# NVIDIA/tensorrt-laboratory

Hardware: NVIDIA H100
Metric: ResNet-50 fp16 b=8 inferences/sec (higher is better)
Workload: dtype f16

## Files before the change

__graft_entry__.py:

```python
from __future__ import annotations

import os
import re
import shutil
import subprocess
import sysconfig
import sys

ROOT = os.path.dirname(os.path.abspath(__file__))
PKG = os.path.join(ROOT, "tensorrt_laboratory_b200")
CSRC = os.path.join(PKG, "csrc")
LIB = os.path.join(PKG, "libb200infer.so")

NVCC_FLAGS = [
    "-gencode", "arch=compute_90a,code=sm_90a", "-lineinfo", "-O3", "-std=c++17",
    "-Xcompiler", "-fPIC,-Wall,-Wno-unused-function", "-cudart", "static",
]


def _nvcc() -> str:
    for cand in (os.environ.get("NVCC"), shutil.which("nvcc"), "/usr/local/cuda/bin/nvcc"):
        if cand and os.path.exists(cand):
            return cand
    raise RuntimeError("nvcc not found")
# ... 20 lines not shown

def _all_deps():
    deps = []
    for root, _, files in os.walk(CSRC):
        deps += [os.path.join(root, f) for f in files if f.endswith((".cu", ".cc", ".h", ".cuh", ".hpp"))]
    deps.append(os.path.join(ROOT, "include", "b200infer.h"))
    inc = os.path.join(ROOT, "include")
    for root, _, files in os.walk(inc):
        deps += [os.path.join(root, f) for f in files]
    return deps


_CONV_KERNEL = re.compile(r"conv|net_f16_tcgen05|attention_f16_wgmma|embed_ln|layernorm_h8|pooler")


_SHARED_SM_KERNEL = re.compile(r"_ZN3b2k(?:16conv_f16_tcgen05|20conv3x3_halo_tcgen05)ILi(\d+)E")
_SHARED_SM_THREADS = 320


def _shared_sm_register_budget(bn: int):
    ctas = 3 if bn <= 64 else 2 if bn <= 128 else 1
    return None if ctas == 1 else 65536 // (_SHARED_SM_THREADS * ctas) // 8 * 8


def _ptxas_violations(log: str):
    bad = [line.strip() for line in log.splitlines() if "(C7520)" in line or "(C7518)" in line]
    func = None
    for line in log.splitlines():
        m = re.search(r"Function properties for (\S+)", line)
        if m:
            func = m.group(1)
# ... 93 lines not shown
```

tensorrt_laboratory_b200/csrc/engine.cu:

```cuda
#include <cuda.h>
#include <cuda_runtime.h>
#include <stdarg.h>
#include <stdio.h>
#include <stdlib.h>
#include <string.h>

#include <algorithm>
#include <map>
#include <memory>
#include <mutex>
#include <string>
#include <vector>

#include "../../include/b200infer.h"
#include "kernels.h"
#include "plan_format.h"

#include "b2_internal.h"

namespace b2i {
thread_local std::string g_err;
int fail(int code, const char* fmt, ...) {
    char buf[1024];
    va_list ap;
// ... 237 lines not shown
    uint8_t* scratch = nullptr;
    struct ScratchState {
        std::map<int, std::unique_ptr<Plan>> plans;
    };
    std::map<uint8_t*, ScratchState> states;
    ScratchState* cur = nullptr;
    int* d_counters = nullptr;
    int use_graph = 1;
    int force_simt = 0;
    int force_im2col = 0;
    int force_bn = 0;
    int force_stages = 0;
    int force_splits = 0;
    int force_sps = 0;
    int force_halo = 0;
    int force_cn = 0;
    int force_ws = 0;
    int pdl_trigger = 1;
    int no_fold = 0;
    int autotune = 4;
    int fork = 0;
    int net = 0;
    int net_ctas = 0;
    int net_bn = 0;
    int net_stages = 0;
    int i8_bn = 0;
    int i8_stages = 0;
    int fuse_tail = 1;
    int input_ctas = 0;
    int* d_tail_ctrl = nullptr;
// ... 301 lines not shown
            return fail(B2_EINVAL, "plan: tactic table outside the blob");
        for (uint32_t i = 0; i < h.n_tactics; ++i) {
            TacticRec t;
            memcpy(&t, base + h.tactics_offset + size_t(i) * sizeof(TacticRec), sizeof t);
            if (t.op >= h.n_ops || t.batch == 0 || t.batch > h.max_batch) return fail(B2_EINVAL, "plan: tactic %u out of range", i);
            ConvConfig cfg{int(t.bn), int(t.stages), int(t.splits), 0.0, int(t.sps), int(t.ws), int(t.cn)};
            cfg.halo = int(t.halo);
            e->tuned[{int(t.op), int(t.batch)}] = cfg;
        }
        e->tactics_from_plan = true;
    }
    *payload = base + h.payload_offset;
    return B2_OK;
}

void plan_arena(b2_engine* e) {
    int busy_until = -1;
    for (size_t i = 0; i < e->ops.size(); ++i) {
        Op& op = e->ops[i];
        op.side_join = -1;
        if (int(i) <= busy_until || op.r.type != b2plan::OP_CONV || op.r.out < 0 || e->tensors[op.r.out].binding >= 0) continue;
        int consumers = 0, join = -1;
        bool as_residual_only = true;
        for (size_t k = i + 1; k < e->ops.size(); ++k) {
            const auto& rk = e->ops[k].r;
            if (rk.in == op.r.out) ++consumers, as_residual_only = false;
            if (rk.res == op.r.out) ++consumers, join = int(k);
        }
        if (consumers == 1 && as_residual_only && join > int(i) + 1) {
            op.side_join = join;
            busy_until = join;
        }
    }
    for (size_t i = 0; i < e->ops.size(); ++i) {
        const auto& r = e->ops[i].r;
        for (int t : {r.out, e->ops[i].out2})
            if (t >= 0 && e->tensors[t].def < 0) e->tensors[t].def = int(i);
        for (int t : {r.in, r.res})
            if (t >= 0) e->tensors[t].last_use = std::max(e->tensors[t].last_use, int(i));
        if (e->ops[i].side_join >= 0 && r.in >= 0) e->tensors[r.in].last_use = std::max(e->tensors[r.in].last_use, e->ops[i].side_join);
    }
    struct Live {
        size_t off, size;
        int last;
    };
    std::vector<Live> live;
    size_t top = 0;
    std::vector<int> order;
    for (size_t i = 0; i < e->tensors.size(); ++i)
        if (e->tensors[i].binding < 0 && e->tensors[i].def >= 0) order.push_back(int(i));
    std::stable_sort(order.begin(), order.end(), [&](int a, int b) { return e->tensors[a].def < e->tensors[b].def; });
    for (int ti : order) {
        Tensor& t = e->tensors[ti];
        if (t.last_use < t.def) t.last_use = t.def;
        const size_t size = align_up(t.item_bytes * e->max_batch, 1024);
// ... 108 lines not shown
    const b2plan::OpRec& r = op.r;
    return !c->no_fold && r.cin_phys == 8 && op.kw() * 8 * 2 == 64 && op.sw() == 1 && op.pw_lo() == 0 && op.pw_hi() == 0;
}
int conv_kb(const b2_context* c, const Op& op) {
    if (op.r.cin_phys % 64 == 0) return 64;
    return conv_is_row_folded(c, op) ? 32 : 8;
}
int conv_num_kblocks(const b2_context* c, const Op& op) {
    const b2plan::OpRec& r = op.r;
    if (op.group_span()) return int(r.taps) * (op.group_span() / 64);
    if (r.cin_phys % 64 == 0) return int(r.taps) * (int(r.cin_phys) / 64);
    if (conv_is_row_folded(c, op)) return (op.kh() + 1) / 2;
    return (int(r.taps_phys) + 7) / 8;
}

int conv_halo_rows(const b2_context* c, const Op& op) {
    const b2plan::OpRec& r = op.r;
    const Tensor& ti = c->e->tensors[r.in];
    const Tensor& to = c->e->tensors[r.out];
    if (op.groups > 1 || r.cin_phys % 64 || r.cout_phys % 64 || op.kh() != 3 || op.kw() != 3 || op.sh() != 1 || op.sw() != 1 || op.ph() != 1 ||
        op.pw_lo() != 1 || op.pw_hi() != 1 || r.res >= 0 || !(r.relu & 2) || ti.h != to.h || ti.w != to.w)
        return 0;
    const int wp = int(to.w) + 2;
    if (wp > 128) return 0;
    return std::min(128 / wp, int(to.h));
}

bool conv_on_tensor_cores(const b2_engine* e, const Op& op) {
    const b2plan::OpRec& r = op.r;
    const bool kb64 = r.cin_phys % 64 == 0, kb8 = r.cin_phys == 8;
    return e->half() && (kb64 || kb8) && r.cout_phys % 32 == 0 && (kb64 || r.taps_phys % 2 == 0) && (op.groups == 1 || op.group_span() > 0);
}

bool conv_takes_stem_ws(const b2_context* c, const Op& op) {
    const b2plan::OpRec& r = op.r;
    return conv_is_row_folded(c, op) && op.kh() == 7 && op.sh() == 2 && r.cout_phys == 64 && c->e->tensors[r.out].w <= 128 &&
           (r.relu & b2plan::kConvRelu) && !(r.relu & 2) && !(r.relu & b2plan::kConvGelu) && r.res < 0 && op.groups == 1;
}

bool conv_takes_ws(const b2_context* c, const Op& op) {
    return conv_takes_stem_ws(c, op) || (conv_kb(c, op) == 64 && (op.r.relu & 2) && op.groups == 1 && !(op.r.relu & b2plan::kConvGelu));
}

bool tactic_applies(const b2_context* c, const Op& op, int batch, const ConvConfig& cfg) {
    const b2plan::OpRec& r = op.r;
    const Tensor& to = c->e->tensors[r.out];
    const int span = op.group_span(), kb = conv_kb(c, op);
    if (cfg.bn <= 0 || int(r.cout_phys) % cfg.bn || cfg.splits < 1 || cfg.sps < 1 || cfg.ws < 0) return false;
    if (op.groups > 1 && (!span || span % cfg.bn || cfg.splits > 1)) return false;
    if ((op.groups > 1 || (r.relu & b2plan::kConvGelu)) && (cfg.ws || cfg.cn > 1 || cfg.halo)) return false;
    if (cfg.halo) {
        const int R = conv_halo_rows(c, op), cblocks = int(r.cin_phys) / 64;
        return R && cfg.splits == 1 && !cfg.ws && cfg.cn <= 1 && b2k::conv_halo_config_exists(cfg.bn) && cblocks <= 8 &&
               b2k::conv_halo_smem(cfg.bn, int(to.w), R, cblocks) <= kSmemLimit;
    }
    if (cfg.ws && conv_is_row_folded(c, op))
        return conv_takes_stem_ws(c, op) && cfg.bn == 64 && cfg.stages == b2k::kStemWsRing && cfg.sps == 1 && cfg.splits == 1 &&
               cfg.cn <= 1 && b2k::conv_stem_ws_smem() <= kSmemLimit;
    if (cfg.ws)
        return conv_takes_ws(c, op) && cfg.splits == 1 && cfg.cn <= 1 && b2k::conv_ws_config_exists(cfg.bn, cfg.stages, cfg.sps) &&
               b2k::conv_ws_smem(cfg.bn, cfg.stages, cfg.sps, r.res >= 0) <= kSmemLimit;
    if (!b2k::conv_config_exists(cfg.bn, kb, cfg.stages, cfg.sps) || b2k::conv_smem_bytes(cfg.bn, cfg.stages, r.res >= 0, cfg.sps) > kSmemLimit)
        return false;
    const int grid_n = int(r.cout_phys) / cfg.bn;
    if (cfg.cn > 1 && (kb != 64 || grid_n % cfg.cn || !b2k::conv_cluster_config_exists(cfg.bn, cfg.stages, cfg.sps, cfg.cn))) return false;
    if (cfg.splits > 1) {
        const int nkb = conv_num_kblocks(c, op), kpc = (nkb + cfg.splits - 1) / cfg.splits;
        const int tiles = (batch * int(to.h * to.w) + 127) / 128 * grid_n;
        if (kb != 64 || kpc < 4 || (cfg.splits - 1) * kpc >= nkb || tiles > kMaxSplitTiles ||
            size_t(tiles) * cfg.splits * 128 * cfg.bn * 4 > kSplitWorkspaceBytes)
            return false;
    }
    return true;
}

std::vector<ConvConfig> conv_candidates(const b2_context* c, const Op& op, int batch, int fixed_splits) {
    const b2plan::OpRec& r = op.r;
    const int kbsz = conv_kb(c, op), nkb = conv_num_kblocks(c, op);
    const int m_tiles = (batch * int(c->e->tensors[r.out].h * c->e->tensors[r.out].w) + 127) / 128;
    const bool ws_only = c->force_ws > 0 && conv_takes_ws(c, op);
    auto ok = [&](const ConvConfig& t) { return tactic_applies(c, op, batch, t); };
    std::vector<ConvConfig> out;
    for (int bn : {256, 128, 64, 32}) {
        if (int(r.cout_phys) % bn) continue;
        const int tiles = m_tiles * (int(r.cout_phys) / bn);
        for (int ws = 0; ws <= 1; ++ws)
        for (int sp : {1, 2, 4, 8})
        for (int sps = 1; sps <= 2; ++sps)
// ... 115 lines not shown
    a.pad_h = op.ph();
    a.pad_w = op.pw_lo();
    a.relu = int(r.relu & (b2plan::kConvRelu | b2plan::kConvGelu));
    a.wpacked = (r.relu & 2) ? w : nullptr;
    const bool tiled = r.k == 1 && op.kw() == 1 && r.stride == 1 && op.sw() == 1 && r.pad_ == 0 && op.pw_lo() == 0 &&
                       op.pw_hi() == 0 && kb64 && (!c->force_im2col || gelu);
    a.a_mode = tiled ? b2k::A_TILED : b2k::A_IM2COL;
    if (cfg.halo) {
        const int R = conv_halo_rows(c, op);
        cl.halo = 1;
        cl.ws_ctas = 0, cl.cn = 1, a.cn = 1, a.splits = 1, cl.stages = kHaloStagesTag, cl.sps = 1;
        a.halo_rows = R;
        cl.grid_m = batch * ((int(to.h) + R - 1) / R);
        int rc = make_map_nhwc(&cl.mapA, tptr(r.in), int(r.cin_phys), int(ti.w), int(ti.h), batch, uint32_t(ti.w) + 2, uint32_t(R) + 2);
        if (rc) return rc;
        rc = make_map_nhwc(&cl.mapOut, tptr(r.out), int(r.cout_phys), int(to.w), int(to.h), batch, uint32_t(to.w) + 2, uint32_t(R));
        cl.mapB = cl.mapA, cl.mapRes = cl.mapOut;
        return rc;
    }
    const CUtensorMapSwizzle swz = kb64 ? CU_TENSOR_MAP_SWIZZLE_128B : (fold ? CU_TENSOR_MAP_SWIZZLE_64B : CU_TENSOR_MAP_SWIZZLE_NONE);
    const uint64_t pix = uint64_t(r.cin_phys) * 2, rowb = uint64_t(ti.w) * pix, imgb = uint64_t(ti.h) * rowb;
    int rc;
    if (tiled)
        rc = make_map_2d(&cl.mapA, tptr(r.in), r.cin_phys, uint64_t(M), 64, uint32_t(128 / cl.cn), swz);
    else if (fold)
        rc = make_map_im2col(&cl.mapA, tptr(r.in), int(r.cin_phys) * op.kw(), int(ti.w) - op.kw() + 1, int(ti.h), batch, pix,
                             rowb, imgb, op.kh(), 1, op.sh(), 1, op.ph(), 0, 0, 32, 128, swz);
    else
        rc = make_map_im2col(&cl.mapA, tptr(r.in), int(r.cin_phys), int(ti.w), int(ti.h), batch, pix, rowb, imgb, op.kh(),
                             op.kw(), op.sh(), op.sw(), op.ph(), op.pw_lo(), op.pw_hi(), uint32_t(cl.kb), uint32_t(128 / cl.cn), swz);
    if (rc) return rc;
    if (r.relu & 2)
// ... 264 lines not shown
        const bool no_split = side || op.groups > 1;
        static const bool tune_splitk = env_int("B2_TUNE_SPLITK", 0) != 0;
        int splits = (no_split || !tune_splitk) ? 1 : 0;
        if (batch != e->max_batch && !no_split && tune_splitk) {
            std::lock_guard<std::mutex> lock(e->tune_mutex);
            auto it = e->tuned.find({int(i), e->max_batch});
            if (it != e->tuned.end()) splits = it->second.splits;
        }
        ConvConfig cfg = pick_conv_config(batch * int(to.h) * int(to.w), int(r.cout_phys), nkb, kbsz, r.res >= 0, c, false,
                                          op.group_span());
        int rc = autotune_conv(c, op, batch, splits, &cfg);
        if (rc) return rc;
        std::lock_guard<std::mutex> lock(e->tune_mutex);
        e->tuned[{int(i), batch}] = cfg;
        tune_cache_append(e, int(i), batch, cfg);
    }
    return B2_OK;
}

int fuse_net_runs(b2_context* c, Plan* plan, int batch) {
    b2_engine* e = c->e;
    std::vector<Launch>& ls = plan->launches;
    bool any = false;
    for (const Launch& L : ls) any = any || L.net_member;
    if (!any) return B2_OK;
    std::vector<Launch> fused;
    size_t i = 0;
    while (i < ls.size()) {
        if (!ls[i].net_member) {
            fused.push_back(std::move(ls[i]));
// ... 110 lines not shown
        run->ctas = std::max(1, std::min(run->ctas, std::min(2 * g_sms, tile_cursor)));
        run->first_op = int(i), run->last_op = int(j);
        Launch L;
        L.kind = L_NET;
        L.name = ls[i].name + ".." + ls[j].name;
        L.flops = flops, L.bytes = bytes;
        L.N = batch;
        L.net = run;
        fused.push_back(std::move(L));
        i = j + 1;
    }
    for (Launch& L : fused) L.side_join = -1;
    ls = std::move(fused);
    plan->has_net = true;
    return B2_OK;
}

void fuse_tail(b2_context* c, Plan* plan, int batch) {
    if (!c->fuse_tail || !c->e->half()) return;
    std::vector<Launch>& ls = plan->launches;
    for (size_t i = 0; i + 2 < ls.size(); ++i) {
        const Launch &P = ls[i], &F = ls[i + 1], &S = ls[i + 2];
        if (P.kind != L_AVGPOOL || F.kind != L_FC || S.kind != L_SOFTMAX) continue;
        if (F.in != P.out || S.in != F.out || F.out_binding >= 0 || S.in_binding >= 0 || S.out_binding < 0 || P.C_phys % 8) continue;
        if (F.K != P.C_phys || S.C != F.Cout || !b2k::tail_f16_applies(batch, P.H * P.W, P.C_phys, F.Cout)) continue;
        Launch T;
        T.kind = L_TAIL;
        T.name = P.name + "+" + F.name + "+" + S.name;
        T.N = batch;
        T.flops = F.flops, T.bytes = P.bytes + F.bytes + S.bytes;
// ... 112 lines not shown
                                        c->force_ws <= 0 && c->force_cn <= 0 && c->force_halo <= 0 && !c->force_im2col && op.groups == 1 &&
                                        !(r.relu & b2plan::kConvGelu);
                    if (net_ok) {
                        int bn = (r.cout_phys % 128 == 0) ? 128 : 64;
                        if (c->net_bn == 64) bn = 64;
                        cfg = ConvConfig{bn, 4, 1, 0.0, 1, 0, 1};
                        cfg.halo = 0;
                        L.net_member = true;
                    } else if (!forced && c->autotune) {
                        std::lock_guard<std::mutex> lock(e->tune_mutex);
                        tune_cache_load(e);
                        auto it = e->tuned.find({op_index, batch});
                        if (it == e->tuned.end()) it = e->tuned.find({op_index, e->max_batch});
                        if (it != e->tuned.end() && tactic_applies(c, op, batch, it->second)) cfg = it->second;
                    }
                    if (op.side_join >= 0 && cfg.splits > 1) cfg.splits = 1;
                    int rc = make_conv_launch(c, op, batch, cfg, &L.conv);
                    if (rc) return rc;
                } else {
                    L.kind = L_CONV_SIMT;
                    b2k::SimtConvArgs& a = L.simt;
                    memset(&a, 0, sizeof a);
                    a.in = tptr(r.in), a.w = w, a.bias = bias;
                    a.residual = r.res >= 0 ? tptr(r.res) : nullptr;
                    a.out = tptr(r.out);
                    a.N = batch, a.H = int(ti.h), a.W = int(ti.w), a.Cin = int(r.cin), a.Cin_phys = int(r.cin_phys);
                    a.Ho = int(to.h), a.Wo = int(to.w), a.Cout = int(r.cout), a.Cout_phys = int(r.cout_phys);
                    a.kh = op.kh(), a.kw = op.kw(), a.taps_phys = int(r.taps_phys);
                    a.stride_h = op.sh(), a.stride_w = op.sw(), a.pad_h = op.ph(), a.pad_w = op.pw_lo();
                    a.relu = int(r.relu & (b2plan::kConvRelu | b2plan::kConvGelu));
// ... 97 lines not shown
                L.in = tptr(r.in);
                L.out = tptr(r.out);
                L.out_binding = to.binding;
                L.w = e->d_payload + r.w_off;
                L.bias = reinterpret_cast<const float*>(e->d_payload + r.b_off);
                L.W = int(ti.w), L.C = int(ti.c), L.C_phys = int(ti.c_phys);
                L.flops = 2.0 * batch * ti.c * ti.c;
                L.bytes = double(r.w_bytes) + double(batch) * (ti.c * 2.0 + to.item_bytes);
                break;
            }
            default:
                return fail(B2_EINVAL, "op %s: unknown type", op.name.c_str());
        }
        plan->launches.push_back(std::move(L));
    }
    int rc = fuse_net_runs(c, plan.get(), batch);
    if (rc) return rc;
    fuse_tail(c, plan.get(), batch);
    {
        const std::vector<Launch>& ls = plan->launches;
        size_t i = 0;
        while (i < ls.size()) {
            const bool dep = ls[i].in_binding >= 0 || ls[i].out_binding >= 0;
            size_t j = i + 1;
            if (!dep)
                while (j < ls.size() && ls[j].in_binding < 0 && ls[j].out_binding < 0) ++j;
            Segment sg;
            sg.begin = int(i), sg.end = int(j);
            sg.graphable = !dep && (j - i) >= 3 && !plan->has_net;
            plan->segments.push_back(sg);
// ... 386 lines not shown
int b2_context_create(b2_engine* e, b2_context** out) {
    if (!e || !out) return fail(B2_EINVAL, "null engine or out");
    if (e->inspect_only) return fail(B2_ESTATE, "engine was loaded with b2_engine_inspect (no device resources)");
    b2_context* c = new b2_context();
    c->e = e;
    c->use_graph = env_int("B2_GRAPH", 1);
    c->force_simt = env_int("B2_FORCE_SIMT", 0);
    c->force_im2col = env_int("B2_FORCE_IM2COL", 0);
    c->force_bn = env_int("B2_FORCE_BN", 0);
    c->force_stages = env_int("B2_FORCE_STAGES", 0);
    c->force_splits = env_int("B2_FORCE_SPLITS", 0);
    c->force_sps = env_int("B2_FORCE_SPS", 0);
    c->force_ws = env_int("B2_FORCE_WS", 0);
    c->force_cn = env_int("B2_FORCE_CN", 0);
    c->force_halo = env_int("B2_FORCE_HALO", 0);
    c->pdl_trigger = env_int("B2_PDL_TRIGGER", 1);
    c->autotune = env_int("B2_AUTOTUNE", 4);
    c->fork = env_int("B2_FORK", 0);
    c->net = env_int("B2_NET", 0);
    c->net_ctas = env_int("B2_NET_CTAS", 0);
    c->net_bn = env_int("B2_NET_BN", 0);
    c->net_stages = env_int("B2_NET_STAGES", 0);
    c->fuse_tail = env_int("B2_FUSE_TAIL", 1);
    c->input_ctas = env_int("B2_INPUT_CTAS", 0);
    c->i8_bn = env_int("B2_I8_BN", 0);
    c->i8_stages = env_int("B2_I8_STAGES", 0);
    if (getenv("B2_PDL")) b2k::set_pdl(env_int("B2_PDL", 1) != 0);
    void* p = nullptr;
    if (cudaMalloc(&p, (kMaxSplitTiles + 16) * sizeof(int)) != cudaSuccess || cudaMemset(p, 0, (kMaxSplitTiles + 16) * sizeof(int)) != cudaSuccess) {
        cudaGetLastError();
// ... 37 lines not shown
        c->use_graph = value;
        return B2_OK;
    }
    if (k == "pdl") {
        b2k::set_pdl(value != 0);
        value = 0;
    } else if (k == "simt") c->force_simt = value;
    else if (k == "im2col") c->force_im2col = value;
    else if (k == "bn") c->force_bn = value;
    else if (k == "stages") c->force_stages = value;
    else if (k == "splits") c->force_splits = value;
    else if (k == "sps") c->force_sps = value;
    else if (k == "ws") c->force_ws = value;
    else if (k == "cn") c->force_cn = value;
    else if (k == "halo") c->force_halo = value;
    else if (k == "fork") c->fork = value;
    else if (k == "net") c->net = value;
    else if (k == "net_ctas") c->net_ctas = value;
    else if (k == "net_bn") c->net_bn = value;
    else if (k == "net_stages") c->net_stages = value;
    else if (k == "fuse_tail") c->fuse_tail = value;
    else if (k == "i8_bn") c->i8_bn = value;
    else if (k == "i8_stages") c->i8_stages = value;
    else if (k == "input_ctas") c->input_ctas = value;
    else if (k == "pdl_trigger") c->pdl_trigger = value;
    else if (k == "autotune") c->autotune = value;
    else if (k == "no_fold") c->no_fold = value;
    else return fail(B2_EINVAL, "unknown option '%s'", key);
    drop_cached(c);
    return B2_OK;
// ... 146 lines not shown
            if (env_int("B2_TUNE_SPLITK", 0) != 0 && !(op.side_join >= 0) && op.groups == 1 && cur.splits == 1 && !cur.halo) {
                const int m_tiles = (batch * int(e->tensors[r.out].h * e->tensors[r.out].w) + 127) / 128;
                for (int sp : {2, 4}) {
                    const int tiles = m_tiles * (int(r.cout_phys) / cur.bn);
                    if (nkb < 16 || tiles >= 100 || tiles * sp > 160 || tiles > kMaxSplitTiles / 8) continue;
                    for (int st : {2, 4})
                        if (tactic_applies(ctx[0].c, op, batch, ConvConfig{cur.bn, st, sp, 0.0, 1, 0, 1}))
                            cands.push_back(ConvConfig{cur.bn, st, sp, 0.0, 1, 0, 1});
                }
            }
            if (cur.splits > 1) continue;
            for (const ConvConfig& t : conv_candidates(ctx[0].c, op, batch, 1))
                if (!t.ws && t.cn <= 1 && t.splits == 1 &&
                    !(t.bn == cur.bn && t.stages == cur.stages && t.sps == cur.sps && t.halo == cur.halo))
                    cands.push_back(t);
            ConvConfig best = cur;
            for (const ConvConfig& cand : cands) {
                {
                    std::lock_guard<std::mutex> lock(e->tune_mutex);
                    e->tuned[{int(i), batch}] = cand;
                }
                const double t = measure();
                if (status) break;
                if (t < base * keep) base = t, best = cand, ++changed;
            }
            std::lock_guard<std::mutex> lock(e->tune_mutex);
            e->tuned[{int(i), batch}] = best;
        }
        if (!changed) break;
    }
// ... 177 lines not shown
    return B2_OK;
}

const char* b2_context_launch_name(b2_context* c, int batch, int i) {
    static thread_local std::string s;
    const Launch* L = get_launch(c, batch, i);
    if (!L) return nullptr;
    static const char* kinds[] = {"input_cast", "conv_tcgen05", "conv_simt", "maxpool", "avgpool", "fc", "softmax", "output_cast", "net_tcgen05", "tail_pool_fc_softmax",
                                  "quantize", "conv_i8_tcgen05", "avgpool_i8", "output_cast_i8", "embed_ln", "layernorm", "attention_f16_wgmma",
                                  "pooler", "output_cast_rows"};
    s = std::string(kinds[L->kind]) + (L->kind == L_ATTENTION && L->attn.S > 128 ? "_ks" : "") + ":" + L->name;
    if (L->kind == L_CONV_TC)
        s += " bn=" + std::to_string(L->conv.bn) + " kb=" + std::to_string(L->conv.kb) +
             " st=" + std::to_string(L->conv.stages) + "x" + std::to_string(L->conv.sps) +
             (L->conv.ws_ctas ? " ws=" + std::to_string(L->conv.ws_ctas) : std::string()) +
             (L->conv.cn > 1 ? " cn=" + std::to_string(L->conv.cn) : std::string()) + (L->conv.halo ? " halo" : "") +
             (L->conv.args.a_mode == b2k::A_TILED ? " tiled" : " im2col") +
             " grid=" + std::to_string(L->conv.grid_n) + "x" + std::to_string(L->conv.grid_m) + "x" +
             std::to_string(L->conv.args.splits) + " kblk=" + std::to_string(L->conv.args.num_kblocks) +
             (L->conv.args.group_span ? " span=" + std::to_string(L->conv.args.group_span) : std::string()) +
             ((L->conv.args.relu & b2plan::kConvGelu) ? " gelu" : "");
    if (L->kind == L_CONV_I8)
        s += " bn=" + std::to_string(L->i8.bn) + " st=" + std::to_string(L->i8.stages) + (L->i8.args.a_mode == b2k::A_TILED ? " tiled" : " im2col") + " grid=" +
             std::to_string(L->i8.grid_n) + "x" + std::to_string(L->i8.grid_m) + " kblk=" + std::to_string(L->i8.args.num_kblocks);
    if (L->kind == L_NET)
        s += " layers=" + std::to_string(L->net->args.n_layers) + " tiles=" + std::to_string(L->net->args.total_tiles) +
             " ctas=" + std::to_string(L->net->ctas) + " stages=" + std::to_string(L->net->args.stages);
    if (L->side_join >= 0) s += " side";
    return s.c_str();
}
double b2_context_launch_flops(b2_context* c, int batch, int i) {
// ... 10 lines not shown
```

tensorrt_laboratory_b200/csrc/kernels.cu:

```cuda
#include "kernels.h"

#include <stdio.h>
#include <stdlib.h>
#include <string.h>

#include <array>
#include <map>
#include <mutex>

#include "ptx_sm90.cuh"
#include "wgmma_sm90.cuh"

namespace b2k {

template <int BN, int STAGES, int SPS = 1>
struct ConvCfg {
    static constexpr int A_SUBBLK = 128 * 64 * 2;
    static constexpr int B_SUBBLK = BN * 64 * 2;
    static constexpr int A_STAGE = SPS * A_SUBBLK;
    static constexpr int B_STAGE = SPS * B_SUBBLK;
    static constexpr int PIPE_BYTES = STAGES * (A_STAGE + B_STAGE);
    static constexpr int TILE_BYTES = 128 * BN * 2;
    static_assert(TILE_BYTES <= PIPE_BYTES, "the output staging tile reuses the pipeline buffers");
};
// ... 926 lines not shown
                    v1 = fmaxf(v1, 0.0f);
                }
                *reinterpret_cast<__half2*>(sOut + so) = __floats2half2_rn(v0, v1);
            }
        }
    }
    fence_proxy_async();
    __syncthreads();
    if (threadIdx.x == kActWarp * 32) {
#pragma unroll
        for (int b = 0; b < NBOX; ++b) tma_store_4d(&mapOut, sOut + b * (128 * 128), n0 + b * OW, 0, h0, img);
        tma_store_commit_and_wait_read();
    }
}

static bool g_use_pdl = true;
void set_pdl(bool on) { g_use_pdl = on; }
bool get_pdl() { return g_use_pdl; }

template <typename Kern, typename... Args>
static int launch_kernel_cluster(Kern kern, dim3 grid, dim3 block, size_t smem, cudaStream_t stream, bool pdl, unsigned cluster_x,
                                 Args... args) {
    cudaLaunchConfig_t cfg = {};
    cfg.gridDim = grid;
    cfg.blockDim = block;
    cfg.dynamicSmemBytes = smem;
    cfg.stream = stream;
    cudaLaunchAttribute attr[2];
    unsigned n = 0;
    if (pdl && g_use_pdl) {
// ... 73 lines not shown

#define B2_FOR_EACH_CONV(X) \
    X(32, 64, 1, 1) X(32, 64, 2, 1) X(32, 64, 4, 1) X(32, 64, 8, 1) \
    X(64, 64, 1, 1) X(64, 64, 2, 1) X(64, 64, 4, 1) X(64, 64, 8, 1) \
    X(128, 64, 1, 1) X(128, 64, 2, 1) X(128, 64, 4, 1) X(256, 64, 2, 1) X(256, 64, 4, 1) \
    X(32, 64, 2, 2) X(32, 64, 4, 2) X(64, 64, 2, 2) X(64, 64, 4, 2) X(128, 64, 2, 2) X(256, 64, 2, 2) \
    X(32, 8, 2, 1) X(32, 8, 4, 1) X(64, 8, 2, 1) X(64, 8, 4, 1) X(64, 8, 8, 1) X(128, 8, 4, 1) \
    X(32, 32, 2, 1) X(32, 32, 4, 1) X(64, 32, 1, 1) X(64, 32, 2, 1) X(64, 32, 4, 1) X(128, 32, 2, 1) X(128, 32, 4, 1)

int conv_halo_smem(int bn, int w, int r, int cblocks) { return halo_smem_bytes(bn, w, r, cblocks); }
bool conv_halo_config_exists(int bn) { return bn == 64 || bn == 128 || bn == 256; }
static int init_conv_halo_kernels() {
    int e;
    if ((e = set_conv_smem(conv3x3_halo_tcgen05<64>, 227 * 1024))) return e;
    if ((e = set_conv_smem(conv3x3_halo_tcgen05<128>, 227 * 1024))) return e;
    return set_conv_smem(conv3x3_halo_tcgen05<256>, 227 * 1024);
}
static int launch_conv_halo(const ConvLaunch& L, cudaStream_t stream) {
    const int R = L.args.halo_rows;
    const size_t smem = size_t(halo_smem_bytes(L.bn, L.args.Wo, R, L.args.cblocks));
    if (smem > 227 * 1024 || R < 1 || R * (L.args.Wo + 2) > 128 || L.args.cblocks > kHaloMaxCBlocks) return static_cast<int>(cudaErrorInvalidValue);
    dim3 grid(L.grid_n, L.grid_m, 1);
    switch (L.bn) {
        case 64: return launch_kernel(conv3x3_halo_tcgen05<64>, grid, dim3(kConvThreads), smem, stream, true, L.mapA, L.mapOut, L.args);
        case 128: return launch_kernel(conv3x3_halo_tcgen05<128>, grid, dim3(kConvThreads), smem, stream, true, L.mapA, L.mapOut, L.args);
        case 256: return launch_kernel(conv3x3_halo_tcgen05<256>, grid, dim3(kConvThreads), smem, stream, true, L.mapA, L.mapOut, L.args);
    }
    return static_cast<int>(cudaErrorInvalidValue);
}

#define B2_FOR_EACH_CONV_CLUSTER(X) \
    X(32, 4, 1, 2) X(32, 4, 1, 4) X(64, 1, 1, 2) X(64, 2, 1, 2) X(64, 2, 1, 4) X(64, 2, 2, 2) X(64, 4, 2, 2) X(64, 4, 2, 4) \
    X(128, 2, 1, 2) X(128, 2, 1, 4) X(128, 2, 2, 2)
// ... 935 lines not shown
```

tensorrt_laboratory_b200/csrc/kernels.h:

```cpp
#pragma once
#include <cuda.h>
#include <cuda_fp16.h>
#include <cuda_runtime.h>
#include <stdint.h>

namespace b2k {

enum { A_TILED = 0, A_IM2COL = 1 };

struct ConvArgs {
    const float* bias;
    const __half* residual;
    __half* out;
    int M;
    int Cout;
    int num_kblocks;
    int cblocks;
    int taps;
    int taps_phys;
    int kw;
    int HoWo, Wo;
    int stride_h, stride_w;
    int pad_h, pad_w;
    int relu;
    int a_mode;
    int splits;
    int kb_per_split;
    float* workspace;
    int* tile_counters;
    int pdl_trigger;
    const uint8_t* wpacked;
    int halo_rows;
    int cn;
    int tiles_m, tiles_n;
    int dbg_mode;
    long long* dbg;
    int group_span;
};

struct ConvLaunch {
    CUtensorMap mapA;
    CUtensorMap mapB;
    CUtensorMap mapOut;
    CUtensorMap mapRes;
    ConvArgs args;
    int bn;
    int kb;
    int stages;
    int sps;
    int grid_m, grid_n;
    int cn;
    int halo;
    int ws_ctas;
};

int launch_conv_f16_tcgen05(const ConvLaunch& L, cudaStream_t stream);
int init_conv_kernels();
bool conv_config_exists(int bn, int kb, int stages, int sps = 1);
int conv_smem_bytes(int bn, int stages, bool residual, int sps = 1);
bool conv_cluster_config_exists(int bn, int stages, int sps, int cn);
bool conv_halo_config_exists(int bn);
int conv_halo_smem(int bn, int w, int r, int cblocks);
int conv_residency(int bn, int kb, int stages, int sps, bool residual, int halo_w = 0, int halo_rows = 0, int cblocks = 0);
bool conv_ws_config_exists(int bn, int stages, int sps);
int conv_ws_smem(int bn, int stages, int sps, bool residual);
constexpr int kStemWsRing = 16;
int conv_stem_ws_smem();
void set_pdl(bool on);
bool get_pdl();

constexpr int kNetMaxLayers = 160;

struct NetLayerInfo {
    const uint8_t* wpacked;
    const float* bias;
    __half* out;
    const __half* residual;
// ... 129 lines not shown
```

Baseline: 31860.

## Fuse bottleneck 3x3 halo conv with following 1x1 residual conv

Adds a fused kernel that computes a 3x3 halo convolution, keeps its activated output in shared memory, and immediately runs the following 1x1 convolution with residual add and ReLU, storing only the final tensor. The aim is to skip writing and re-reading the intermediate activation and to save one launch per ResNet bottleneck. The fused tactic is picked only when the autotuner measures it faster than the two separate convs, or when forced by an environment flag. It adds plan rewriting, arena lifetime changes and a larger shared-memory footprint, which may reduce occupancy.

```diff
diff --git a/__graft_entry__.py b/__graft_entry__.py
--- a/__graft_entry__.py
+++ b/__graft_entry__.py
@@ -58,7 +58,7 @@
 _CONV_KERNEL = re.compile(r"conv|net_f16_tcgen05|attention_f16_wgmma|embed_ln|layernorm_h8|pooler")
 
 
-_SHARED_SM_KERNEL = re.compile(r"_ZN3b2k(?:16conv_f16_tcgen05|20conv3x3_halo_tcgen05)ILi(\d+)E")
+_SHARED_SM_KERNEL = re.compile(r"_ZN3b2k(?:16conv_f16_tcgen05|20conv3x3_halo_tcgen05|24conv3x3_halo_1x1_tcgen05)ILi(\d+)E")
 _SHARED_SM_THREADS = 320
 
 
diff --git a/tensorrt_laboratory_b200/csrc/engine.cu b/tensorrt_laboratory_b200/csrc/engine.cu
--- a/tensorrt_laboratory_b200/csrc/engine.cu
+++ b/tensorrt_laboratory_b200/csrc/engine.cu
@@ -275,6 +275,7 @@
     int force_splits = 0;
     int force_sps = 0;
     int force_halo = 0;
+    int force_fuse = 0;
     int force_cn = 0;
     int force_ws = 0;
     int pdl_trigger = 1;
@@ -606,6 +607,8 @@
     return B2_OK;
 }
 
+int fuse_partner(const b2_engine* e, int i);
+
 void plan_arena(b2_engine* e) {
     int busy_until = -1;
     for (size_t i = 0; i < e->ops.size(); ++i) {
@@ -631,6 +634,8 @@
         for (int t : {r.in, r.res})
             if (t >= 0) e->tensors[t].last_use = std::max(e->tensors[t].last_use, int(i));
         if (e->ops[i].side_join >= 0 && r.in >= 0) e->tensors[r.in].last_use = std::max(e->tensors[r.in].last_use, e->ops[i].side_join);
+        const int j = fuse_partner(e, int(i));
+        if (j >= 0) e->tensors[r.in].last_use = std::max(e->tensors[r.in].last_use, j);
     }
     struct Live {
         size_t off, size;
@@ -769,16 +774,37 @@
     return (int(r.taps_phys) + 7) / 8;
 }
 
-int conv_halo_rows(const b2_context* c, const Op& op) {
+int conv_halo_rows(const b2_engine* e, const Op& op) {
     const b2plan::OpRec& r = op.r;
-    const Tensor& ti = c->e->tensors[r.in];
-    const Tensor& to = c->e->tensors[r.out];
+    const Tensor& ti = e->tensors[r.in];
+    const Tensor& to = e->tensors[r.out];
     if (op.groups > 1 || r.cin_phys % 64 || r.cout_phys % 64 || op.kh() != 3 || op.kw() != 3 || op.sh() != 1 || op.sw() != 1 || op.ph() != 1 ||
         op.pw_lo() != 1 || op.pw_hi() != 1 || r.res >= 0 || !(r.relu & 2) || ti.h != to.h || ti.w != to.w)
         return 0;
     const int wp = int(to.w) + 2;
     if (wp > 128) return 0;
     return std::min(128 / wp, int(to.h));
+}
+int conv_halo_rows(const b2_context* c, const Op& op) { return conv_halo_rows(c->e, op); }
+bool conv_on_tensor_cores(const b2_engine* e, const Op& op);
+
+int fuse_partner(const b2_engine* e, int i) {
+    if (!e->half() || e->int8() || i < 0 || size_t(i) + 1 >= e->ops.size()) return -1;
+    const Op &oi = e->ops[size_t(i)], &oj = e->ops[size_t(i) + 1];
+    const b2plan::OpRec &ri = oi.r, &rj = oj.r;
+    if (ri.type != b2plan::OP_CONV || rj.type != b2plan::OP_CONV || (ri.relu & (4 | b2plan::kConvGelu)) || conv_halo_rows(e, oi) == 0 ||
+        !b2k::conv_halo_config_exists(int(ri.cout_phys)) || ri.cin_phys / 64 > 8)
+        return -1;
+    if (rj.in != ri.out || rj.res < 0 || rj.res == ri.out || oj.kh() != 1 || oj.kw() != 1 || oj.sh() != 1 || oj.sw() != 1 || oj.ph() != 0 ||
+        oj.pw_lo() != 0 || oj.pw_hi() != 0 || oj.groups != 1 || !(rj.relu & 2) || (rj.relu & (4 | b2plan::kConvGelu)) ||
+        rj.cin_phys != ri.cout_phys || rj.cout_phys % 64 || !conv_on_tensor_cores(e, oj) || e->tensors[ri.out].binding >= 0)
+        return -1;
+    for (size_t k = 0; k < e->ops.size(); ++k) {
+        const b2plan::OpRec& rk = e->ops[k].r;
+        if (k != size_t(i) + 1 && (rk.in == ri.out || rk.res == ri.out || e->ops[k].out2 == ri.out)) return -1;
+        if (k == size_t(i) + 1 && rk.res == ri.out) return -1;
+    }
+    return i + 1;
 }
 
 bool conv_on_tensor_cores(const b2_engine* e, const Op& op) {
@@ -804,9 +830,15 @@
     if (cfg.bn <= 0 || int(r.cout_phys) % cfg.bn || cfg.splits < 1 || cfg.sps < 1 || cfg.ws < 0) return false;
     if (op.groups > 1 && (!span || span % cfg.bn || cfg.splits > 1)) return false;
     if ((op.groups > 1 || (r.relu & b2plan::kConvGelu)) && (cfg.ws || cfg.cn > 1 || cfg.halo)) return false;
+    if (cfg.halo == 2) {
+        const int j = fuse_partner(c->e, int(&op - &c->e->ops[0]));
+        const int R = conv_halo_rows(c, op), cblocks = int(r.cin_phys) / 64;
+        return j >= 0 && c->force_fuse >= 0 && cfg.bn == int(r.cout_phys) && cfg.splits == 1 && !cfg.ws && cfg.cn <= 1 &&
+               b2k::conv_halo_fused_smem(cfg.bn, int(to.w), R, cblocks, int(c->e->ops[size_t(j)].r.cout_phys)) <= kSmemLimit;
+    }
     if (cfg.halo) {
         const int R = conv_halo_rows(c, op), cblocks = int(r.cin_phys) / 64;
-        return R && cfg.splits == 1 && !cfg.ws && cfg.cn <= 1 && b2k::conv_halo_config_exists(cfg.bn) && cblocks <= 8 &&
+        return cfg.halo == 1 && R && cfg.splits == 1 && !cfg.ws && cfg.cn <= 1 && b2k::conv_halo_config_exists(cfg.bn) && cblocks <= 8 &&
                b2k::conv_halo_smem(cfg.bn, int(to.w), R, cblocks) <= kSmemLimit;
     }
     if (cfg.ws && conv_is_row_folded(c, op))
@@ -827,6 +859,14 @@
             return false;
     }
     return true;
+}
+
+constexpr int kFuseMinStreams = 4;
+
+ConvConfig fused_conv_config(const Op& op) {
+    ConvConfig f{int(op.r.cout_phys), kHaloStagesTag, 1, 0.0, 1, 0, 1};
+    f.halo = 2;
+    return f;
 }
 
 std::vector<ConvConfig> conv_candidates(const b2_context* c, const Op& op, int batch, int fixed_splits) {
@@ -972,8 +1012,21 @@
         cl.grid_m = batch * ((int(to.h) + R - 1) / R);
         int rc = make_map_nhwc(&cl.mapA, tptr(r.in), int(r.cin_phys), int(ti.w), int(ti.h), batch, uint32_t(ti.w) + 2, uint32_t(R) + 2);
         if (rc) return rc;
+        cl.mapB = cl.mapA;
+        if (cfg.halo == 2) {
+            const Op& oj = e->ops[size_t(fuse_partner(e, int(&op - &e->ops[0])))];
+            const b2plan::OpRec& rj = oj.r;
+            cl.halo = 2;
+            cl.c2.wpacked = e->d_payload + rj.w_off;
+            cl.c2.bias = reinterpret_cast<const float*>(e->d_payload + rj.b_off);
+            cl.c2.Cout = int(rj.cout_phys);
+            cl.c2.relu = int(rj.relu & b2plan::kConvRelu);
+            rc = make_map_nhwc(&cl.mapOut, tptr(rj.out), int(rj.cout_phys), int(to.w), int(to.h), batch, uint32_t(to.w) + 2, uint32_t(R));
+            if (!rc) rc = make_map_nhwc(&cl.mapRes, tptr(rj.res), int(rj.cout_phys), int(to.w), int(to.h), batch, uint32_t(to.w) + 2, uint32_t(R));
+            return rc;
+        }
         rc = make_map_nhwc(&cl.mapOut, tptr(r.out), int(r.cout_phys), int(to.w), int(to.h), batch, uint32_t(to.w) + 2, uint32_t(R));
-        cl.mapB = cl.mapA, cl.mapRes = cl.mapOut;
+        cl.mapRes = cl.mapOut;
         return rc;
     }
     const CUtensorMapSwizzle swz = kb64 ? CU_TENSOR_MAP_SWIZZLE_128B : (fold ? CU_TENSOR_MAP_SWIZZLE_64B : CU_TENSOR_MAP_SWIZZLE_NONE);
@@ -1268,6 +1321,37 @@
         std::lock_guard<std::mutex> lock(e->tune_mutex);
         e->tuned[{int(i), batch}] = cfg;
         tune_cache_append(e, int(i), batch, cfg);
+    }
+    for (size_t i = 0; i < e->ops.size() && c->force_fuse >= 0 && c->autotune >= kFuseMinStreams; ++i) {
+        const Op& op = e->ops[i];
+        const int j = fuse_partner(e, int(i));
+        if (j < 0) continue;
+        double unfused_us = 0;
+        {
+            std::lock_guard<std::mutex> lock(e->tune_mutex);
+            const auto a = e->tuned.find({int(i), batch}), b = e->tuned.find({j, batch});
+            if (a == e->tuned.end() || b == e->tuned.end() || a->second.halo == 2 || !(a->second.est_us > 0) || !(b->second.est_us > 0)) continue;
+            unfused_us = a->second.est_us + b->second.est_us;
+        }
+        ConvConfig f = fused_conv_config(op);
+        if (!tactic_applies(c, op, batch, f)) continue;
+        b2k::ConvLaunch cl;
+        int rc = make_conv_launch(c, op, batch, f, &cl);
+        if (rc) return rc;
+        TuneTimer tt(c);
+        if ((rc = tt.init())) return rc;
+        float ms = 0.f;
+        const cudaError_t err = tt.time([&](int, cudaStream_t s) { return b2k::launch_conv_f16_tcgen05(cl, s); }, &ms);
+        if (err != cudaSuccess) return fail(B2_ECUDA, "autotune of %s fused with %s failed: %s", op.name.c_str(), e->ops[size_t(j)].name.c_str(), cudaGetErrorString(err));
+        f.est_us = tt.us_per_launch(ms);
+        if (env_int("B2_TUNE_VERBOSE", 0))
+            fprintf(stderr, "[b2 tune] %s+%s b=%d fused : %.3f us/launch against %.3f unfused (%d streams) -> %s\n", op.name.c_str(),
+                    e->ops[size_t(j)].name.c_str(), batch, f.est_us, unfused_us, tt.ns, f.est_us < unfused_us ? "fused" : "unfused");
+        if (f.est_us < unfused_us) {
+            std::lock_guard<std::mutex> lock(e->tune_mutex);
+            e->tuned[{int(i), batch}] = f;
+            tune_cache_append(e, int(i), batch, f);
+        }
     }
     return B2_OK;
 }
@@ -1408,6 +1492,32 @@
     ls = std::move(fused);
     plan->has_net = true;
     return B2_OK;
+}
+
+void fuse_bottlenecks(b2_context* c, Plan* plan, int batch) {
+    std::vector<Launch>& ls = plan->launches;
+    if (std::none_of(ls.begin(), ls.end(), [](const Launch& L) { return L.kind == L_CONV_TC && L.conv.halo == 2; })) return;
+    std::vector<int> new_index(ls.size());
+    std::vector<Launch> out;
+    for (size_t k = 0; k < ls.size(); ++k) {
+        new_index[k] = int(out.size());
+        if (ls[k].kind == L_CONV_TC && ls[k].conv.halo == 2 && k + 1 < ls.size()) {
+            Launch& J = ls[k + 1];
+            Launch L = std::move(ls[k]);
+            const Tensor& mid = c->e->tensors[c->e->ops[k].r.out];
+            L.name += "+" + J.name;
+            L.flops += J.flops;
+            L.bytes += J.bytes - 2.0 * batch * double(mid.item_bytes);
+            new_index[k + 1] = new_index[k];
+            ++k;
+            out.push_back(std::move(L));
+            continue;
+        }
+        out.push_back(std::move(ls[k]));
+    }
+    for (Launch& L : out)
+        if (L.side_join >= 0) L.side_join = new_index[size_t(L.side_join)];
+    ls = std::move(out);
 }
 
 void fuse_tail(b2_context* c, Plan* plan, int batch) {
@@ -1550,6 +1660,10 @@
                         if (it == e->tuned.end()) it = e->tuned.find({op_index, e->max_batch});
                         if (it != e->tuned.end() && tactic_applies(c, op, batch, it->second)) cfg = it->second;
                     }
+                    if (!net_ok && c->force_fuse > 0) {
+                        const ConvConfig f = fused_conv_config(op);
+                        if (tactic_applies(c, op, batch, f)) cfg = f;
+                    }
                     if (op.side_join >= 0 && cfg.splits > 1) cfg.splits = 1;
                     int rc = make_conv_launch(c, op, batch, cfg, &L.conv);
                     if (rc) return rc;
@@ -1677,6 +1791,7 @@
         }
         plan->launches.push_back(std::move(L));
     }
+    fuse_bottlenecks(c, plan.get(), batch);
     int rc = fuse_net_runs(c, plan.get(), batch);
     if (rc) return rc;
     fuse_tail(c, plan.get(), batch);
@@ -2093,6 +2208,7 @@
     c->force_ws = env_int("B2_FORCE_WS", 0);
     c->force_cn = env_int("B2_FORCE_CN", 0);
     c->force_halo = env_int("B2_FORCE_HALO", 0);
+    c->force_fuse = env_int("B2_FORCE_FUSE", 0);
     c->pdl_trigger = env_int("B2_PDL_TRIGGER", 1);
     c->autotune = env_int("B2_AUTOTUNE", 4);
     c->fork = env_int("B2_FORK", 0);
@@ -2160,6 +2276,7 @@
     else if (k == "ws") c->force_ws = value;
     else if (k == "cn") c->force_cn = value;
     else if (k == "halo") c->force_halo = value;
+    else if (k == "fuse") c->force_fuse = value;
     else if (k == "fork") c->fork = value;
     else if (k == "net") c->net = value;
     else if (k == "net_ctas") c->net_ctas = value;
@@ -2336,6 +2453,8 @@
                 if (!t.ws && t.cn <= 1 && t.splits == 1 &&
                     !(t.bn == cur.bn && t.stages == cur.stages && t.sps == cur.sps && t.halo == cur.halo))
                     cands.push_back(t);
+            if (streams >= kFuseMinStreams && cur.halo != 2 && tactic_applies(ctx[0].c, op, batch, fused_conv_config(op)))
+                cands.push_back(fused_conv_config(op));
             ConvConfig best = cur;
             for (const ConvConfig& cand : cands) {
                 {
@@ -2543,7 +2662,8 @@
         s += " bn=" + std::to_string(L->conv.bn) + " kb=" + std::to_string(L->conv.kb) +
              " st=" + std::to_string(L->conv.stages) + "x" + std::to_string(L->conv.sps) +
              (L->conv.ws_ctas ? " ws=" + std::to_string(L->conv.ws_ctas) : std::string()) +
-             (L->conv.cn > 1 ? " cn=" + std::to_string(L->conv.cn) : std::string()) + (L->conv.halo ? " halo" : "") +
+             (L->conv.cn > 1 ? " cn=" + std::to_string(L->conv.cn) : std::string()) +
+             (L->conv.halo == 2 ? " halo fused" : L->conv.halo ? " halo" : "") +
              (L->conv.args.a_mode == b2k::A_TILED ? " tiled" : " im2col") +
              " grid=" + std::to_string(L->conv.grid_n) + "x" + std::to_string(L->conv.grid_m) + "x" +
              std::to_string(L->conv.args.splits) + " kblk=" + std::to_string(L->conv.args.num_kblocks) +
diff --git a/tensorrt_laboratory_b200/csrc/kernels.cu b/tensorrt_laboratory_b200/csrc/kernels.cu
--- a/tensorrt_laboratory_b200/csrc/kernels.cu
+++ b/tensorrt_laboratory_b200/csrc/kernels.cu
@@ -964,6 +964,217 @@
     }
 }
 
+constexpr int kFuseChunk = 64;
+constexpr int kFuseTile = 128 * kFuseChunk * 2;
+__host__ __device__ constexpr int halo_fused_smem_bytes(int bn, int w, int r, int cblocks, int cout2) {
+    const int halo = cblocks * halo_a_stage_bytes(w, r), a2 = bn * 256;
+    return (halo > a2 ? halo : a2) + 2 * kFuseTile + halo_b_stages(bn) * bn * 128 + 256 + (bn + cout2) * 4 + 1024;
+}
+
+template <int BN>
+__global__ void __launch_bounds__(kConvThreads, conv_min_ctas(BN))
+conv3x3_halo_1x1_tcgen05(const __grid_constant__ CUtensorMap mapIn, const __grid_constant__ CUtensorMap mapRes,
+                         const __grid_constant__ CUtensorMap mapOut, const ConvArgs p, const Conv1x1Args q) {
+    constexpr int NB = halo_b_stages(BN);
+    constexpr int B_BLK = BN * 128;
+    constexpr int C_BLK = kFuseChunk * 128;
+    constexpr int KB2 = BN / 64;
+
+    extern __shared__ uint8_t smem_raw[];
+    uint8_t* smem = smem_raw + ((1024u - (smem_u32(smem_raw) & 1023u)) & 1023u);
+    const int W = p.Wo, Wp = p.Wo + 2, R = p.halo_rows;
+    const int a_stage = halo_a_stage_bytes(W, R);
+    const int cblocks = p.cblocks;
+    const int region0 = max(cblocks * a_stage, BN * 256);
+    uint8_t* sA = smem;
+    uint8_t* sR = smem + region0;
+    uint8_t* sB = sR + 2 * kFuseTile;
+    uint8_t* tail = sB + NB * B_BLK;
+    uint64_t* a_full = reinterpret_cast<uint64_t*>(tail);
+    uint64_t* b_full = a_full + kHaloMaxCBlocks;
+    uint64_t* b_empty = b_full + NB;
+    uint64_t* r_full = b_empty + NB;
+    uint64_t* e_done = r_full + 2;
+    uint64_t* bias_bar = e_done + 2;
+    float* s_bias = reinterpret_cast<float*>(tail + 256);
+    float* s_bias2 = s_bias + BN;
+
+    const int warp = threadIdx.x >> 5;
+    const int lane = threadIdx.x & 31;
+    const int Ho = p.HoWo / p.Wo;
+    const int tiles_per_img = (Ho + R - 1) / R;
+    const int img = blockIdx.y / tiles_per_img;
+    const int h0 = (blockIdx.y - img * tiles_per_img) * R;
+    const int nsteps = cblocks * 9;
+    const int nchunks = q.Cout / kFuseChunk;
+    const int nsteps_all = nsteps + nchunks * KB2;
+
+    if (threadIdx.x == 0) {
+        tma_prefetch_desc(&mapIn);
+        tma_prefetch_desc(&mapRes);
+        tma_prefetch_desc(&mapOut);
+        for (int s = 0; s < cblocks; ++s) mbar_init(&a_full[s], 1);
+        for (int s = 0; s < NB; ++s) {
+            mbar_init(&b_full[s], 1);
+            mbar_init(&b_empty[s], kConsumerWarps);
+        }
+        for (int s = 0; s < 2; ++s) {
+            mbar_init(&r_full[s], 1);
+            mbar_init(&e_done[s], kConsumerWarps);
+        }
+        mbar_init(bias_bar, 32);
+        fence_barrier_init();
+        fence_proxy_async();
+    }
+    __syncthreads();
+    if (p.pdl_trigger == 0) pdl_launch_dependents();
+
+    if (warp == kActWarp) {
+        const uint32_t box_bytes = static_cast<uint32_t>(R * Wp * 128);
+        auto load_res = [&](int c) {
+            mbar_expect_tx(&r_full[c & 1], box_bytes);
+            tma_load_4d(&mapRes, &r_full[c & 1], sR + (c & 1) * kFuseTile, c * kFuseChunk, 0, h0, img);
+        };
+        pdl_wait();
+        if (elect_one_sync()) {
+            for (int cb = 0; cb < cblocks; ++cb) {
+                mbar_expect_tx(&a_full[cb], static_cast<uint32_t>((R + 2) * Wp * 128));
+                tma_load_4d(&mapIn, &a_full[cb], sA + cb * a_stage, cb * 64, -1, h0 - 1, img);
+            }
+            for (int c = 0; c < 2 && c < nchunks; ++c) load_res(c);
+            for (int c = 0; c < nchunks; ++c) {
+                mbar_wait(&e_done[c & 1], (c >> 1) & 1);
+                tma_store_4d(&mapOut, sR + (c & 1) * kFuseTile, c * kFuseChunk, 0, h0, img);
+                tma_store_commit_and_wait_read();
+                if (c + 2 < nchunks) load_res(c + 2);
+            }
+        }
+        __syncwarp();
+    } else if (warp < kConsumerWarps) {
+        const uint32_t wg = static_cast<uint32_t>(warp >> 2);
+        const uint32_t wg_off = wg * 8192u;
+        float acc[BN / 2];
+        int i = 0;
+#pragma unroll 1
+        for (int tap = 0; tap < 9; ++tap) {
+            const int r = tap / 3, sx = tap - r * 3;
+            const uint32_t tap_off = static_cast<uint32_t>((r * Wp + sx) * 128);
+#pragma unroll 1
+            for (int cb = 0; cb < cblocks; ++cb, ++i) {
+                const int sb = i % NB;
+                if (tap == 0) mbar_wait(&a_full[cb], 0);
+                mbar_wait(&b_full[sb], (i / NB) & 1);
+                const uint32_t a_addr = smem_u32(sA + cb * a_stage) + tap_off + wg_off;
+                const uint32_t b_addr = smem_u32(sB + sb * B_BLK);
+                wgmma_fence();
+#pragma unroll
+                for (int j = 0; j < 4; ++j) {
+                    const uint64_t ad = make_wgmma_desc(a_addr + j * 32, 16, 1024, WG_SW128);
+                    const uint64_t bd = make_wgmma_desc(b_addr + j * 32, 16, 1024, WG_SW128);
+                    wgmma_f16<BN>(acc, ad, bd, (i > 0 || j > 0) ? 1u : 0u);
+                }
+                wgmma_commit();
+                wgmma_wait<1>();
+                __syncwarp();
+                if (i > 0 && lane == 0) mbar_arrive(&b_empty[(i - 1) % NB]);
+            }
+        }
+        wgmma_wait<0>();
+        __syncwarp();
+        if (lane == 0) mbar_arrive(&b_empty[(nsteps - 1) % NB]);
+
+        named_bar_sync(1, kConsumerWarps * 32);
+        mbar_wait(bias_bar, 0);
+        const FragPos fp(warp, lane);
+#pragma unroll
+        for (int j = 0; j < BN / 8; ++j) {
+#pragma unroll
+            for (int h = 0; h < 2; ++h) {
+                const int row = fp.row0 + 8 * h, col = 8 * j + fp.col0;
+                const uint32_t so = static_cast<uint32_t>((col / 64) * (128 * 128)) + swz_off<128>(row, (col % 64) / 8) + (col % 8) * 2;
+                float v0 = acc[4 * j + 2 * h] + s_bias[col], v1 = acc[4 * j + 2 * h + 1] + s_bias[col + 1];
+                if (p.relu) {
+                    v0 = fmaxf(v0, 0.0f);
+                    v1 = fmaxf(v1, 0.0f);
+                }
+                *reinterpret_cast<__half2*>(sA + so) = __floats2half2_rn(v0, v1);
+            }
+        }
+        fence_proxy_async();
+        named_bar_sync(2 + wg, 128);
+
+#pragma unroll 1
+        for (int c = 0; c < nchunks; ++c) {
+            float acc2[kFuseChunk / 2];
+#pragma unroll
+            for (int kb = 0; kb < KB2; ++kb, ++i) {
+                const int sb = i % NB;
+                mbar_wait(&b_full[sb], (i / NB) & 1);
+                const uint32_t a_addr = smem_u32(sA + kb * (128 * 128)) + wg_off;
+                const uint32_t b_addr = smem_u32(sB + sb * B_BLK);
+                wgmma_fence();
+#pragma unroll
+                for (int j = 0; j < 4; ++j) {
+                    const uint64_t ad = make_wgmma_desc(a_addr + j * 32, 16, 1024, WG_SW128);
+                    const uint64_t bd = make_wgmma_desc(b_addr + j * 32, 16, 1024, WG_SW128);
+                    wgmma_f16<kFuseChunk>(acc2, ad, bd, (kb > 0 || j > 0) ? 1u : 0u);
+                }
+                wgmma_commit();
+                wgmma_wait<1>();
+                __syncwarp();
+                if (kb > 0 && lane == 0) mbar_arrive(&b_empty[(i - 1) % NB]);
+            }
+            wgmma_wait<0>();
+            __syncwarp();
+            if (lane == 0) mbar_arrive(&b_empty[(i - 1) % NB]);
+            if (c == nchunks - 1 && p.pdl_trigger == 1) pdl_launch_dependents();
+            uint8_t* buf = sR + (c & 1) * kFuseTile;
+            mbar_wait(&r_full[c & 1], (c >> 1) & 1);
+#pragma unroll
+            for (int j = 0; j < kFuseChunk / 8; ++j) {
+#pragma unroll
+                for (int h = 0; h < 2; ++h) {
+                    const int row = fp.row0 + 8 * h, col = 8 * j + fp.col0;
+                    const uint32_t so = swz_off<128>(row, col / 8) + (col % 8) * 2;
+                    float v0 = acc2[4 * j + 2 * h] + s_bias2[c * kFuseChunk + col];
+                    float v1 = acc2[4 * j + 2 * h + 1] + s_bias2[c * kFuseChunk + col + 1];
+                    const float2 rf = __half22float2(*reinterpret_cast<const __half2*>(buf + so));
+                    v0 += rf.x;
+                    v1 += rf.y;
+                    if (q.relu) {
+                        v0 = fmaxf(v0, 0.0f);
+                        v1 = fmaxf(v1, 0.0f);
+                    }
+                    *reinterpret_cast<__half2*>(buf + so) = __floats2half2_rn(v0, v1);
+                }
+            }
+            fence_proxy_async();
+            __syncwarp();
+            if (lane == 0) mbar_arrive(&e_done[c & 1]);
+        }
+    } else if (warp == kWgtWarp) {
+        for (int i = lane; i < BN; i += 32) s_bias[i] = __ldg(p.bias + i);
+        for (int i = lane; i < q.Cout; i += 32) s_bias2[i] = __ldg(q.bias + i);
+        mbar_arrive(bias_bar);
+        for (int i = 0; i < nsteps_all; ++i) {
+            const int sb = i % NB;
+            if (i >= NB) mbar_wait(&b_empty[sb], ((i / NB) & 1) ^ 1);
+            if (elect_one_sync()) {
+                if (i < nsteps) {
+                    mbar_expect_tx(&b_full[sb], B_BLK);
+                    bulk_load_1d(&b_full[sb], sB + sb * B_BLK, p.wpacked + static_cast<size_t>(i) * (BN >> 5) * 4096, B_BLK);
+                } else {
+                    const int t = i - nsteps, c = t / KB2, kb = t - c * KB2;
+                    mbar_expect_tx(&b_full[sb], C_BLK);
+                    bulk_load_1d(&b_full[sb], sB + sb * B_BLK,
+                                 q.wpacked + (static_cast<size_t>(kb) * (q.Cout >> 5) + c * (kFuseChunk >> 5)) * 4096, C_BLK);
+                }
+            }
+            __syncwarp();
+        }
+    }
+}
+
 static bool g_use_pdl = true;
 void set_pdl(bool on) { g_use_pdl = on; }
 bool get_pdl() { return g_use_pdl; }
@@ -1067,9 +1278,28 @@
     int e;
     if ((e = set_conv_smem(conv3x3_halo_tcgen05<64>, 227 * 1024))) return e;
     if ((e = set_conv_smem(conv3x3_halo_tcgen05<128>, 227 * 1024))) return e;
-    return set_conv_smem(conv3x3_halo_tcgen05<256>, 227 * 1024);
+    if ((e = set_conv_smem(conv3x3_halo_tcgen05<256>, 227 * 1024))) return e;
+    if ((e = set_conv_smem(conv3x3_halo_1x1_tcgen05<64>, 227 * 1024))) return e;
+    if ((e = set_conv_smem(conv3x3_halo_1x1_tcgen05<128>, 227 * 1024))) return e;
+    return set_conv_smem(conv3x3_halo_1x1_tcgen05<256>, 227 * 1024);
+}
+int conv_halo_fused_smem(int bn, int w, int r, int cblocks, int cout2) { return halo_fused_smem_bytes(bn, w, r, cblocks, cout2); }
+static int launch_conv_halo_fused(const ConvLaunch& L, cudaStream_t stream) {
+    const int R = L.args.halo_rows;
+    const size_t smem = size_t(halo_fused_smem_bytes(L.bn, L.args.Wo, R, L.args.cblocks, L.c2.Cout));
+    if (smem > 227 * 1024 || R < 1 || R * (L.args.Wo + 2) > 128 || L.args.cblocks > kHaloMaxCBlocks || L.grid_n != 1 ||
+        L.bn != L.args.Cout || L.c2.Cout < kFuseChunk || L.c2.Cout % kFuseChunk)
+        return static_cast<int>(cudaErrorInvalidValue);
+    dim3 grid(1, L.grid_m, 1);
+    switch (L.bn) {
+        case 64: return launch_kernel(conv3x3_halo_1x1_tcgen05<64>, grid, dim3(kConvThreads), smem, stream, true, L.mapA, L.mapRes, L.mapOut, L.args, L.c2);
+        case 128: return launch_kernel(conv3x3_halo_1x1_tcgen05<128>, grid, dim3(kConvThreads), smem, stream, true, L.mapA, L.mapRes, L.mapOut, L.args, L.c2);
+        case 256: return launch_kernel(conv3x3_halo_1x1_tcgen05<256>, grid, dim3(kConvThreads), smem, stream, true, L.mapA, L.mapRes, L.mapOut, L.args, L.c2);
+    }
+    return static_cast<int>(cudaErrorInvalidValue);
 }
 static int launch_conv_halo(const ConvLaunch& L, cudaStream_t stream) {
+    if (L.halo == 2) return launch_conv_halo_fused(L, stream);
     const int R = L.args.halo_rows;
     const size_t smem = size_t(halo_smem_bytes(L.bn, L.args.Wo, R, L.args.cblocks));
     if (smem > 227 * 1024 || R < 1 || R * (L.args.Wo + 2) > 128 || L.args.cblocks > kHaloMaxCBlocks) return static_cast<int>(cudaErrorInvalidValue);
diff --git a/tensorrt_laboratory_b200/csrc/kernels.h b/tensorrt_laboratory_b200/csrc/kernels.h
--- a/tensorrt_laboratory_b200/csrc/kernels.h
+++ b/tensorrt_laboratory_b200/csrc/kernels.h
@@ -38,6 +38,13 @@
     int group_span;
 };
 
+struct Conv1x1Args {
+    const uint8_t* wpacked;
+    const float* bias;
+    int Cout;
+    int relu;
+};
+
 struct ConvLaunch {
     CUtensorMap mapA;
     CUtensorMap mapB;
@@ -52,6 +59,7 @@
     int cn;
     int halo;
     int ws_ctas;
+    Conv1x1Args c2;
 };
 
 int launch_conv_f16_tcgen05(const ConvLaunch& L, cudaStream_t stream);
@@ -61,6 +69,7 @@
 bool conv_cluster_config_exists(int bn, int stages, int sps, int cn);
 bool conv_halo_config_exists(int bn);
 int conv_halo_smem(int bn, int w, int r, int cblocks);
+int conv_halo_fused_smem(int bn, int w, int r, int cblocks, int cout2);
 int conv_residency(int bn, int kb, int stages, int sps, bool residual, int halo_w = 0, int halo_rows = 0, int cblocks = 0);
 bool conv_ws_config_exists(int bn, int stages, int sps);
 int conv_ws_smem(int bn, int stages, int sps, bool residual);
```

New measurement: 33150, median of 6. 1.04x the previous value.
